# wkentaro/chainer-mask-rcnn

Hardware: AMD Instinct MI355X
Metric: images/sec train step, ResNet50-C4 Mask R-CNN, COCO 800x1333 (higher is better)
Workload: dtype f32 (bf16x3 split operands, f32 accumulate)

## Files before the change

### chainer_mask_rcnn_amd/csrc/conv_gemm.hip

```cpp
#include <algorithm>
#include <cstring>

#include "conv_gemm_kernel.h"

namespace {

__global__ void splitk_reduce_kernel(const float *__restrict__ ws, int splits, int64_t n,
                                     int64_t stride, float *__restrict__ out)
{
    const int64_t nv = n / 4;
    for (int64_t i = (int64_t)blockIdx.x * blockDim.x + threadIdx.x; i < nv;
         i += (int64_t)gridDim.x * blockDim.x) {
        float4 a = reinterpret_cast<const float4 *>(ws)[i];
        int s = 1;
        for (; s + 4 <= splits; s += 4) {
            const float4 v0 = reinterpret_cast<const float4 *>(ws + (s + 0) * stride)[i];
            const float4 v1 = reinterpret_cast<const float4 *>(ws + (s + 1) * stride)[i];
            const float4 v2 = reinterpret_cast<const float4 *>(ws + (s + 2) * stride)[i];
            const float4 v3 = reinterpret_cast<const float4 *>(ws + (s + 3) * stride)[i];
            a.x += v0.x; a.y += v0.y; a.z += v0.z; a.w += v0.w;
            a.x += v1.x; a.y += v1.y; a.z += v1.z; a.w += v1.w;
            a.x += v2.x; a.y += v2.y; a.z += v2.z; a.w += v2.w;
            a.x += v3.x; a.y += v3.y; a.z += v3.z; a.w += v3.w;
        }
// ... 214 lines not shown
                      (int64_t)d->N * d->P * d->Q * d->K < (int64_t)INT32_MAX,
                  "conv: tensor exceeds 2^31 elements");
    return 0;
}

inline bool aligned16(const void *p) { return ((uintptr_t)p % 16) == 0; }

int set_extents(GemmParams &p, int64_t a_floats, int64_t b_floats, int64_t c_floats)
{
    const int64_t lim = (int64_t)1 << 29;
    MRCNN_REQUIRE(a_floats < lim && b_floats < lim && c_floats < lim,
                  "conv: a tensor exceeds 2 GiB (%lld / %lld / %lld floats); split the batch",
                  (long long)a_floats, (long long)b_floats, (long long)c_floats);
    p.a_bytes = (unsigned)(a_floats * 4);
    p.b_bytes = (unsigned)(b_floats * 4);
    p.c_bytes = (unsigned)(c_floats * 4);
    return 0;
}


int fwd_problem(const mrcnn_conv_desc *d, GemmParams &p)
{
    if (int rc = check_desc(d)) return rc;
    p.M = d->N * d->P * d->Q; p.N = d->K; p.Kc = d->C;
    p.gp = d->P; p.gq = d->Q; p.sh = d->H; p.sw = d->W;
    p.R = d->R; p.S = d->S; p.stride = d->stride; p.pad = d->pad;
    p.lda = d->C; p.ldb = d->R * d->S * d->C; p.ldc = d->K;
    p.out_mode = OUT_PLAIN;
    p.perm_n = choose_perm(g_knobs, d->N, d->P, d->Q, d->R, d->S, d->stride, d->pad);
    if (p.perm_n) p.M = (int)(mrcnn::ceil_div(d->N, kPermBlock) * kPermBlock) * d->P * d->Q;
    return set_extents(p, (int64_t)d->N * d->H * d->W * d->C, (int64_t)d->K * d->R * d->S * d->C,
                       (int64_t)d->N * d->P * d->Q * d->K);
}

int stem_problem(int N, int H, int W, int K, GemmParams &p)
{
    MRCNN_REQUIRE(N > 0 && H > 0 && W > 0 && K > 0 && K % 4 == 0, "conv_stem: bad shape");
    const int P = (H + 6 - 7) / 2 + 1, Q = (W + 6 - 7) / 2 + 1;
    p.M = N * P * Q; p.N = K; p.Kc = 32;
    p.gp = P; p.gq = Q; p.sh = H; p.sw = W;
    p.R = 7; p.S = 1; p.stride = 2; p.pad = 3;
    p.lda = 4; p.ldb = 7 * 32; p.ldc = K;
    p.out_mode = OUT_PLAIN; p.stem = 1;
    return set_extents(p, (int64_t)N * H * W * 4, (int64_t)K * 7 * 32, (int64_t)N * P * Q * K);
}

int dgrad_problem(const mrcnn_conv_desc *d, bool fused_grad, GemmParams &p)
{
    if (int rc = check_desc(d)) return rc;
    MRCNN_REQUIRE(!fused_grad || d->stride == 1,
                  "conv2d_dgrad: residual gradient / output mask need stride 1");
    p.N = d->C; p.Kc = d->K; p.cin = d->C;
    p.R = d->R; p.S = d->S; p.pad = d->pad;
    p.lda = d->K; p.ldb = d->R * d->S * d->C; p.ldc = d->C;
    p.sh = d->P; p.sw = d->Q;
    if (d->stride == 1) {
        p.M = d->N * d->H * d->W; p.gp = d->H; p.gq = d->W; p.stride = 1;
        p.out_mode = OUT_PLAIN;
    } else {
        MRCNN_REQUIRE(d->R == 1 && d->S == 1 && d->pad == 0,
                      "conv2d_dgrad: stride>1 is implemented for 1x1/pad0 (the only strided "
                      "trainable convs of ResNet-C4) and the 2x2/2 adjoint (deconv entry points)");
        p.M = d->N * d->P * d->Q; p.gp = d->P; p.gq = d->Q; p.stride = d->stride;
        p.out_mode = OUT_STRIDED; p.oh = d->H; p.ow = d->W;
    }
    return set_extents(p, (int64_t)d->N * d->P * d->Q * d->K, (int64_t)d->K * d->R * d->S * d->C,
                       (int64_t)d->N * d->H * d->W * d->C);
}

int dgrad_wt_problem(const mrcnn_conv_desc *d, bool fused_grad, GemmParams &p)
{
    if (int rc = check_desc(d)) return rc;
    const bool strided = d->stride > 1;
    MRCNN_REQUIRE(!strided || (d->R == 1 && d->S == 1 && d->pad == 0),
                  "conv2d_dgrad_wt: stride > 1 is implemented for 1x1 / pad 0 filters");
    MRCNN_REQUIRE(!strided || !fused_grad, "conv2d_dgrad_wt: residual gradient / output mask need stride 1");
    p.N = d->C; p.Kc = d->K;
    p.sh = d->P; p.sw = d->Q;
    p.R = d->R; p.S = d->S; p.stride = 1; p.pad = d->R - 1 - d->pad;
    p.lda = d->K; p.ldb = d->R * d->S * d->K; p.ldc = d->C;
    if (strided) {
        p.gp = d->P; p.gq = d->Q; p.ostride = d->stride;
        p.out_mode = OUT_STRIDED; p.oh = d->H; p.ow = d->W;
    } else {
        p.gp = d->H; p.gq = d->W;
        p.out_mode = OUT_PLAIN;
        p.perm_n = choose_perm(g_knobs, d->N, d->H, d->W, d->R, d->S, 1, p.pad);
    }
    p.M = d->N * p.gp * p.gq;
    if (p.perm_n) p.M = (int)(mrcnn::ceil_div(d->N, kPermBlock) * kPermBlock) * d->H * d->W;
    MRCNN_REQUIRE(d->S - 1 - d->pad == p.pad, "conv2d_dgrad_wt: square filters / symmetric padding only");
    return set_extents(p, (int64_t)d->N * d->P * d->Q * d->K, (int64_t)d->K * d->R * d->S * d->C,
                       (int64_t)d->N * d->H * d->W * d->C);
}

int wgrad_problem(const mrcnn_conv_desc *d, GemmParams &p, GemmShape &shape)
{
    const int64_t pixels = (int64_t)d->N * d->P * d->Q;
    p.M = d->K; p.N = d->R * d->S * d->C; p.Kc = (int)pixels;
    p.gp = d->P; p.gq = d->Q; p.sh = d->H; p.sw = d->W;
    p.R = d->R; p.S = d->S; p.stride = d->stride; p.pad = d->pad;
    p.lda = d->C; p.ldg = d->K; p.cin = d->C; p.ldc = d->R * d->S * d->C;
    shape = gemm_shape(p, WGRAD, false);
    shape.pixels = pixels; shape.n_img = d->N; shape.C = d->C;
    return set_extents(p, pixels * d->K, (int64_t)d->N * d->H * d->W * d->C, (int64_t)d->K * d->R * d->S * d->C);
}

inline mrcnn_conv_desc deconv_adjoint_desc(int N, int H, int W, int C, int K)
{
    return {N, 2 * H, 2 * W, K, C, 2, 2, 2, 0, H, W};
}

int deconv_problem(bool wt, int N, int H, int W, int C, int K, GemmParams &p)
{
    MRCNN_REQUIRE(N > 0 && H > 0 && W > 0 && C > 0 && K > 0 && C % 4 == 0 && K % 4 == 0,
                  "%s: bad shape", wt ? "deconv_fwd_wt" : "deconv_fwd");
    p.M = N * H * W; p.N = 4 * K; p.Kc = C; p.cin = wt ? 0 : 4 * K;
    p.gp = H; p.gq = W; p.sh = H; p.sw = W;
    p.R = 1; p.S = 1; p.stride = 1; p.pad = 0;
    p.lda = C; p.ldb = wt ? C : 4 * K; p.ldc = K;
    p.out_mode = OUT_DECONV; p.ko = K;
    return set_extents(p, (int64_t)N * H * W * C, (int64_t)C * 4 * K, (int64_t)N * 4 * H * W * K);
}

int deconv_fwd(bool wt, const float *x, const float *w, const float *bias, float *y, int N, int H, int W,
               int C, int K, int epi_flags, void *stream)
{
    const char *who = wt ? "deconv_fwd_wt" : "deconv_fwd";
    GemmParams p = {};
    if (int rc = deconv_problem(wt, N, H, W, C, K, p)) return rc;
    MRCNN_REQUIRE(x && w && y, "%s: null pointer", who);
    MRCNN_REQUIRE(aligned16(x) && aligned16(w), "%s: x/%s must be 16-byte aligned", who, wt ? "wT" : "w");
    MRCNN_REQUIRE((epi_flags & ~(MRCNN_EPI_BIAS | MRCNN_EPI_RELU)) == 0, "%s: bad flags", who);
    MRCNN_REQUIRE(!(epi_flags & MRCNN_EPI_BIAS) || bias, "%s: bias flag without bias", who);
    p.A = x; p.B = w; p.C = y; p.bias = bias;
    p.flags = epi_flags;
    return wt ? launch<FWD>(p, mrcnn::as_stream(stream)) : launch<DGRAD>(p, mrcnn::as_stream(stream));
}

int wgrad_run(const mrcnn_conv_desc *d, const float *gy, const float *x, float *gw, void *ws,
              const float *out_row_scale, void *stream)
{
    GemmParams p = {};
    GemmShape shape;
    if (int rc = wgrad_problem(d, p, shape)) return rc;
    p.A = gy; p.B = x; p.C = gw;
    p.scale = out_row_scale;
    p.split_ws = (float *)ws;
    shape.has_ws = ws != nullptr;
    return run_plan<WGRAD>(p, plan_wgrad(shape, g_knobs), mrcnn::as_stream(stream));
}

extern float g_wino_ambiguity;

}

extern "C" int64_t mrcnn_conv2d_split_workspace_bytes(void) { return kSplitWsBytes; }

extern "C" int mrcnn_set_tuning(const char *name, int value)
{
    MRCNN_REQUIRE(name != nullptr, "set_tuning: null name");
    MRCNN_REQUIRE(knob_value_ok(name, value), "set_tuning: split_planes must be 1, 2 or 3, got %d (it stays %d)",
                  value, g_knobs.split_planes);
    if (set_knob(g_knobs, name, value)) return 0;
    if (strcmp(name, "wino_ambiguity_ppb") == 0) {
        g_wino_ambiguity = 1e-9f * (float)value;
        return 0;
    }
    if (int rc = mrcnn::roi_align_set_tuning(name, value); rc >= 0) return rc;
    MRCNN_REQUIRE(false, "set_tuning: unknown option '%s'", name);
    return 1;
}

extern "C" int mrcnn_conv2d_fwd(const mrcnn_conv_desc *d, const float *x, const float *w,
                                const float *bias, const float *scale, const float *shift,
                                const float *residual, float *y, int epi_flags, void *split_ws,
                                void *stream)
{
    GemmParams p = {};
    if (int rc = fwd_problem(d, p)) return rc;
    MRCNN_REQUIRE(x && w && y, "conv2d_fwd: null pointer");
    MRCNN_REQUIRE(aligned16(x) && aligned16(w), "conv2d_fwd: x/w must be 16-byte aligned");
    MRCNN_REQUIRE(!(epi_flags & MRCNN_EPI_BIAS) || bias, "conv2d_fwd: bias flag without bias");
    MRCNN_REQUIRE(!(epi_flags & MRCNN_EPI_AFFINE) || (scale && shift), "conv2d_fwd: affine flag without scale/shift");
    MRCNN_REQUIRE(!(epi_flags & MRCNN_EPI_RESIDUAL) || residual, "conv2d_fwd: residual flag without residual");
    p.A = x; p.B = w; p.C = y;
    p.bias = bias; p.scale = scale; p.shift = shift; p.residual = residual;
    p.flags = epi_flags;
    p.split_ws = (float *)split_ws;
    return launch<FWD>(p, mrcnn::as_stream(stream));
}

extern "C" int mrcnn_conv_stem_fwd(const float *x4, const float *w784, const float *bias,
                                   const float *scale, const float *shift, float *y, int N, int H,
                                   int W, int K, int epi_flags, void *stream)
{
    GemmParams p = {};
    if (int rc = stem_problem(N, H, W, K, p)) return rc;
    MRCNN_REQUIRE(x4 && w784 && y, "conv_stem: null pointer");
    MRCNN_REQUIRE(aligned16(x4) && aligned16(w784), "conv_stem: pointers must be 16-byte aligned");
    p.A = x4; p.B = w784; p.C = y;
    p.bias = bias; p.scale = scale; p.shift = shift;
    p.flags = epi_flags;
    return launch<FWD>(p, mrcnn::as_stream(stream));
}

extern "C" int mrcnn_conv2d_dgrad_ex(const mrcnn_conv_desc *d, const float *gy, const float *w,
                                     float *gx, int epi_flags, const float *res_g,
                                     const float *res_y, const float *out_mask_y,
                                     const float *out_scale, void *split_ws, void *stream)
{
    GemmParams p = {};
    if (int rc = dgrad_problem(d, res_g || out_mask_y, p)) return rc;
    MRCNN_REQUIRE(!res_y || res_g, "conv2d_dgrad: res_y without res_g");
    MRCNN_REQUIRE(gy && w && gx, "conv2d_dgrad: null pointer");
    MRCNN_REQUIRE(aligned16(gy) && aligned16(w), "conv2d_dgrad: gy/w must be 16-byte aligned");
    MRCNN_REQUIRE((epi_flags & ~MRCNN_EPI_ACCUM) == 0, "conv2d_dgrad: only MRCNN_EPI_ACCUM is valid");
    hipStream_t s = mrcnn::as_stream(stream);
    p.A = gy; p.B = w; p.C = gx;
    p.res_g = res_g; p.res_y = res_y; p.out_mask_y = out_mask_y; p.scale = out_scale;
    p.flags = epi_flags | (out_scale ? MRCNN_EPI_AFFINE : 0);
    p.split_ws = (float *)split_ws;
    if (p.out_mode == OUT_STRIDED && !(epi_flags & MRCNN_EPI_ACCUM))
        MRCNN_HIP_TRY(hipMemsetAsync(gx, 0, sizeof(float) * (size_t)d->N * d->H * d->W * d->C, s));
    return launch<DGRAD>(p, s);
}

extern "C" int mrcnn_conv2d_dgrad(const mrcnn_conv_desc *d, const float *gy, const float *w,
                                  float *gx, int epi_flags, void *stream)
{
    return mrcnn_conv2d_dgrad_ex(d, gy, w, gx, epi_flags, nullptr, nullptr, nullptr, nullptr, nullptr,
                                 stream);
}


namespace {
__global__ void filter_flip_transpose_kernel(const float *__restrict__ w, float *__restrict__ wT,
                                             int K, int RS, int C,
                                             const float *__restrict__ row_scale)
{
    __shared__ float tile[32][33];
    const int rs = blockIdx.z;
    const int k0 = blockIdx.y * 32, c0 = blockIdx.x * 32;
    const int tx = threadIdx.x & 31, ty = threadIdx.x >> 5;
    for (int j = ty; j < 32; j += 8) {
        const int k = k0 + j, c = c0 + tx;
        tile[j][tx] = (k < K && c < C)
                          ? w[((int64_t)k * RS + rs) * C + c] * (row_scale ? row_scale[k] : 1.f)
                          : 0.f;
    }
    __syncthreads();
    for (int j = ty; j < 32; j += 8) {
        const int c = c0 + j, k = k0 + tx;
        if (c < C && k < K) wT[((int64_t)c * RS + (RS - 1 - rs)) * K + k] = tile[tx][j];
    }
}

constexpr int kFlipBatch = 32;
struct FlipBatch {
    const float *w[kFlipBatch];
    float *wT[kFlipBatch];
    const float *scale[kFlipBatch];
    int K[kFlipBatch], RS[kFlipBatch], C[kFlipBatch];
    int first_block[kFlipBatch + 1];
    int n;
};

__global__ void filter_flip_transpose_batched_kernel(const FlipBatch b)
{
    __shared__ float tile[32][33];
    int l = 0;
    while (l + 1 < b.n && (int)blockIdx.x >= b.first_block[l + 1]) ++l;
    const int K = b.K[l], RS = b.RS[l], C = b.C[l];
    int blk = blockIdx.x - b.first_block[l];
    const int ncb = (C + 31) / 32, nkb = (K + 31) / 32;
    const int cb = blk % ncb;
    blk /= ncb;
    const int kb = blk % nkb, rs = blk / nkb;
    const float *__restrict__ w = b.w[l];
    float *__restrict__ wT = b.wT[l];
    const float *__restrict__ row_scale = b.scale[l];
    const int k0 = kb * 32, c0 = cb * 32;
    const int tx = threadIdx.x & 31, ty = threadIdx.x >> 5;
    for (int j = ty; j < 32; j += 8) {
        const int k = k0 + j, c = c0 + tx;
        tile[j][tx] = (k < K && c < C)
                          ? w[((int64_t)k * RS + rs) * C + c] * (row_scale ? row_scale[k] : 1.f)
                          : 0.f;
    }
    __syncthreads();
    for (int j = ty; j < 32; j += 8) {
        const int c = c0 + j, k = k0 + tx;
        if (c < C && k < K) wT[((int64_t)c * RS + (RS - 1 - rs)) * K + k] = tile[tx][j];
    }
}
}

extern "C" int mrcnn_filter_flip_transpose_batched(int n, const void *const *w, void *const *wT,
                                                   const int *K, const int *R, const int *S,
                                                   const int *C, const void *const *row_scale,
                                                   void *stream)
{
    MRCNN_REQUIRE(n >= 0 && (n == 0 || (w && wT && K && R && S && C)),
                  "filter_flip_transpose_batched: bad args");
    for (int i0 = 0; i0 < n; i0 += kFlipBatch) {
        FlipBatch b = {};
        b.n = std::min(kFlipBatch, n - i0);
        int blocks = 0;
        for (int i = 0; i < b.n; ++i) {
            const int j = i0 + i;
            MRCNN_REQUIRE(w[j] && wT[j] && K[j] > 0 && R[j] > 0 && S[j] > 0 && C[j] > 0,
                          "filter_flip_transpose_batched: bad entry %d", j);
            b.w[i] = (const float *)w[j];
            b.wT[i] = (float *)wT[j];
            b.scale[i] = row_scale ? (const float *)row_scale[j] : nullptr;
            b.K[i] = K[j]; b.RS[i] = R[j] * S[j]; b.C[i] = C[j];
            b.first_block[i] = blocks;
            blocks += ((C[j] + 31) / 32) * ((K[j] + 31) / 32) * R[j] * S[j];
        }
// ... 176 lines not shown
```

### chainer_mask_rcnn_amd/csrc/conv_winograd.h

```cpp
#pragma once

namespace {

constexpr int kXi = 36;

struct F2 { float x, y; };
__device__ __forceinline__ F2 operator+(F2 a, F2 b) { return {a.x + b.x, a.y + b.y}; }
__device__ __forceinline__ F2 operator-(F2 a, F2 b) { return {a.x - b.x, a.y - b.y}; }
__device__ __forceinline__ F2 operator*(float s, F2 a) { return {s * a.x, s * a.y}; }

template <typename T>
__device__ __forceinline__ void wino_bt(const T (&d)[6], T (&t)[6])
{
    t[0] = d[0] - 1.5f * d[1] - 2.f * d[2] + 1.5f * d[3] + d[4];
    t[1] = 2.5f * d[3] + 0.5f * d[2] - d[1] + d[4];
    t[2] = d[1] - 2.5f * d[2] + 0.5f * d[3] + d[4];
    t[3] = 2.f * (d[3] - d[1]) - d[2] + d[4];
    t[4] = 0.5f * (d[1] - d[3]) - d[2] + d[4];
    t[5] = d[1] - 1.5f * d[2] - 2.f * d[3] + 1.5f * d[4] + d[5];
}
template <typename T>
__device__ __forceinline__ void wino_at(const T (&m)[6], T (&y)[4])
{
    const T s12 = m[1] + m[2], d12 = m[1] - m[2];
    y[0] = m[0] + s12 + m[3] + m[4];
    y[1] = d12 + 0.5f * m[3] - 2.f * m[4];
    y[2] = s12 + 0.25f * m[3] + 4.f * m[4];
    y[3] = d12 + 0.125f * m[3] - 8.f * m[4] + m[5];
}
template <typename T>
__device__ __forceinline__ void wino_at_abs(const T (&m)[6], T (&y)[4])
{
    const T s12 = m[1] + m[2];
    y[0] = m[0] + s12 + m[3] + m[4];
    y[1] = s12 + 0.5f * m[3] + 2.f * m[4];
    y[2] = s12 + 0.25f * m[3] + 4.f * m[4];
    y[3] = s12 + 0.125f * m[3] + 8.f * m[4] + m[5];
}
template <typename T>
__device__ __forceinline__ void wino_g4(const T (&g)[4], T (&t)[6])
{
    t[0] = g[0];
    t[1] = g[0] + g[1] + g[2] + g[3];
    t[2] = g[1] - g[0] - g[2] + g[3];
    t[3] = -16.f * g[0] - 8.f * g[1] - 4.f * g[2] - 2.f * g[3];
    t[4] = g[0] - 2.f * g[1] + 4.f * g[2] - 8.f * g[3];
    t[5] = g[3];
}

__constant__ double kFilterG[6][3] = {{1., 0., 0.},
                                      {1. / 3, 1. / 3, 1. / 3},
                                      {-1. / 3, 1. / 3, -1. / 3},
                                      {-16. / 15, -8. / 15, -4. / 15},
                                      {1. / 15, -2. / 15, 4. / 15},
                                      {0., 0., 1.}};
__constant__ double kWgradAT[3][6] = {{1., 1. / 3, 1. / 3, 1. / 15, 1. / 15, 0.},
                                      {0., 1. / 3, -1. / 3, 1. / 30, -2. / 15, 0.},
                                      {0., 1. / 3, 1. / 3, 1. / 60, 4. / 15, 1.}};

struct WinoGeom {
    int N, H, W, TH, TW;
    int64_t T;
};
inline WinoGeom wino_geom(const mrcnn_conv_desc *d)
{
    WinoGeom g;
    g.N = d->N; g.H = d->H; g.W = d->W;
    g.TH = (d->H + 3) / 4; g.TW = (d->W + 3) / 4;
    g.T = (int64_t)d->N * g.TH * g.TW;
    return g;
}

template <bool GRAD_TILE>
__global__ void __launch_bounds__(256) wino_data_transform_kernel(
    const float *__restrict__ x, float *__restrict__ v, int H, int W, int C, int TH, int TW,
    int64_t T)
{
    constexpr int D = GRAD_TILE ? 4 : 6;
    const int c2n = C >> 1;
    const int64_t idx = (int64_t)blockIdx.x * 256 + threadIdx.x;
    if (idx >= T * c2n) return;
    const int64_t tile = idx / c2n;
    const int c = (int)(idx - tile * c2n) * 2;
    const int tx = (int)(tile % TW);
    const int64_t q = tile / TW;
    const int ty = (int)(q % TH);
    const int64_t n = q / TH;
    const int y0 = 4 * ty - (GRAD_TILE ? 0 : 1), x0 = 4 * tx - (GRAD_TILE ? 0 : 1);
    const float *base = x + (n * H * W) * C + c;
    F2 d[D][D];
#pragma unroll
    for (int i = 0; i < D; ++i)
#pragma unroll
        for (int j = 0; j < D; ++j) {
            const int yy = y0 + i, xx = x0 + j;
            const bool ok = (unsigned)yy < (unsigned)H && (unsigned)xx < (unsigned)W;
            d[i][j] = ok ? *reinterpret_cast<const F2 *>(base + ((int64_t)yy * W + xx) * C)
                         : F2{0.f, 0.f};
        }
    F2 t[6][D];
#pragma unroll
    for (int j = 0; j < D; ++j) {
        F2 col[D], o[6];
#pragma unroll
        for (int i = 0; i < D; ++i) col[i] = d[i][j];
        if constexpr (GRAD_TILE) wino_g4(col, o);
        else wino_bt(col, o);
#pragma unroll
        for (int a = 0; a < 6; ++a) t[a][j] = o[a];
    }
    float *out = v + tile * C + c;
    const int64_t xi_stride = T * C;
#pragma unroll
    for (int a = 0; a < 6; ++a) {
        F2 o[6];
        if constexpr (GRAD_TILE) wino_g4(t[a], o);
        else wino_bt(t[a], o);
#pragma unroll
        for (int b = 0; b < 6; ++b)
            *reinterpret_cast<F2 *>(out + (a * 6 + b) * xi_stride) = o[b];
    }
}

struct WinoOutParams {
    const float *m;
    float *y;
    const float *scale, *shift, *mask;
    int H, W, K, TH, TW, flags;
    int64_t T;
    int *fix_count;
    int2 *fix_list;
    int fix_cap;
    float ambiguity;
};
float g_wino_ambiguity = 4e-6f;

template <bool FIXUP>
__global__ void __launch_bounds__(256) wino_output_transform_kernel(const WinoOutParams p)
{
    const int k2n = p.K >> 1;
    const int64_t idx = (int64_t)blockIdx.x * 256 + threadIdx.x;
    if (idx >= p.T * k2n) return;
    const int64_t tile = idx / k2n;
    const int k = (int)(idx - tile * k2n) * 2;
    const int tx = (int)(tile % p.TW);
    const int64_t q = tile / p.TW;
    const int ty = (int)(q % p.TH);
    const int64_t n = q / p.TH;
    const float *in = p.m + tile * p.K + k;
    const int64_t xi_stride = p.T * p.K;
    F2 m[6][6];
#pragma unroll
    for (int a = 0; a < 6; ++a)
#pragma unroll
        for (int b = 0; b < 6; ++b)
            m[a][b] = *reinterpret_cast<const F2 *>(in + (a * 6 + b) * xi_stride);
    const int y0 = 4 * ty, x0 = 4 * tx;
    const int64_t obase = (n * p.H * p.W) * p.K + k;
    F2 mk[4][4];
    if (p.mask) {
#pragma unroll
        for (int i = 0; i < 4; ++i)
#pragma unroll
            for (int j = 0; j < 4; ++j) {
                const bool ok = y0 + i < p.H && x0 + j < p.W;
                mk[i][j] = ok ? *reinterpret_cast<const F2 *>(
                                    p.mask + obase + ((int64_t)(y0 + i) * p.W + x0 + j) * p.K)
                              : F2{0.f, 0.f};
            }
    }
    F2 s[4][6];
    F2 sa[FIXUP ? 4 : 1][6];
#pragma unroll
    for (int b = 0; b < 6; ++b) {
        F2 col[6], o[4];
#pragma unroll
        for (int a = 0; a < 6; ++a) col[a] = m[a][b];
        wino_at(col, o);
#pragma unroll
        for (int i = 0; i < 4; ++i) s[i][b] = o[i];
        if constexpr (FIXUP) {
#pragma unroll
            for (int a = 0; a < 6; ++a) col[a] = F2{fabsf(col[a].x), fabsf(col[a].y)};
            wino_at_abs(col, o);
#pragma unroll
            for (int i = 0; i < 4; ++i) sa[i][b] = o[i];
        }
    }
    F2 sc = {1.f, 1.f}, sh = {0.f, 0.f};
    const bool aff = (p.flags & (MRCNN_EPI_AFFINE | MRCNN_EPI_BIAS)) != 0;
    const bool relu = (p.flags & MRCNN_EPI_RELU) != 0;
    if (aff) {
        if (p.scale) sc = *reinterpret_cast<const F2 *>(p.scale + k);
        if (p.shift) sh = *reinterpret_cast<const F2 *>(p.shift + k);
    }
#pragma unroll
    for (int i = 0; i < 4; ++i) {
        F2 o[4], ob[4];
        wino_at(s[i], o);
        if constexpr (FIXUP) wino_at_abs(sa[i], ob);
#pragma unroll
        for (int j = 0; j < 4; ++j) {
            if (y0 + i >= p.H || x0 + j >= p.W) continue;
            F2 v = o[j];
            if (aff) { v.x = v.x * sc.x + sh.x; v.y = v.y * sc.y + sh.y; }
            if constexpr (FIXUP) {
                const float bx = p.ambiguity * ob[j].x * fabsf(sc.x);
                const float by = p.ambiguity * ob[j].y * fabsf(sc.y);
                const int pix = (int)(n * p.H * p.W) + (y0 + i) * p.W + x0 + j;
                if (fabsf(v.x) < bx) {
                    const int at = atomicAdd(p.fix_count, 1);
                    if (at < p.fix_cap) p.fix_list[at] = make_int2(pix, k);
                }
                if (fabsf(v.y) < by) {
                    const int at = atomicAdd(p.fix_count, 1);
                    if (at < p.fix_cap) p.fix_list[at] = make_int2(pix, k + 1);
                }
            }
            if (relu) { v.x = fmaxf(v.x, 0.f); v.y = fmaxf(v.y, 0.f); }
            if (p.mask) {
                v.x = mk[i][j].x > 0.f ? v.x : 0.f;
                v.y = mk[i][j].y > 0.f ? v.y : 0.f;
            }
            *reinterpret_cast<F2 *>(p.y + obase + ((int64_t)(y0 + i) * p.W + x0 + j) * p.K) = v;
        }
    }
}

struct WinoFixParams {
    const float *x, *w, *scale, *shift;
    float *y;
    const int *count;
    const int2 *list;
    int cap, H, W, C, K, flags;
};
__global__ void __launch_bounds__(256) wino_fixup_kernel(const WinoFixParams p)
{
    const int lane = threadIdx.x & 63;
    const int wave = (int)((blockIdx.x * 256 + threadIdx.x) >> 6), nwaves = (int)(gridDim.x * 4);
    const int n_items = min(*p.count, p.cap);
    for (int it = wave; it < n_items; it += nwaves) {
        const int2 e = p.list[it];
        const int pix = e.x, k = e.y;
        const int n = pix / (p.H * p.W), rem = pix - n * (p.H * p.W);
        const int yy = rem / p.W, xx = rem - yy * p.W;
        float acc = 0.f;
        for (int r = 0; r < 3; ++r) {
            const int iy = yy + r - 1;
            if ((unsigned)iy >= (unsigned)p.H) continue;
            for (int s = 0; s < 3; ++s) {
                const int ix = xx + s - 1;
                if ((unsigned)ix >= (unsigned)p.W) continue;
                const float *xp = p.x + ((int64_t)(n * p.H + iy) * p.W + ix) * p.C;
                const float *wp = p.w + ((int64_t)k * 9 + r * 3 + s) * p.C;
                for (int c = lane * 4; c < p.C; c += 256) {
                    const float4 a = *reinterpret_cast<const float4 *>(xp + c);
                    const float4 b = *reinterpret_cast<const float4 *>(wp + c);
                    acc += (a.x * b.x + a.y * b.y) + (a.z * b.z + a.w * b.w);
                }
            }
        }
#pragma unroll
        for (int off = 32; off > 0; off >>= 1) acc += __shfl_down(acc, off, 64);
        if (lane == 0) {
            float v = acc;
            if (p.flags & (MRCNN_EPI_AFFINE | MRCNN_EPI_BIAS))
                v = v * (p.scale ? p.scale[k] : 1.f) + (p.shift ? p.shift[k] : 0.f);
            if (p.flags & MRCNN_EPI_RELU) v = fmaxf(v, 0.f);
            p.y[(int64_t)pix * p.K + k] = v;
        }
    }
}

template <bool TRANSPOSED>
__global__ void __launch_bounds__(256) wino_filter_transform_kernel(
    const float *__restrict__ w, float *__restrict__ u, int K, int C,
    const float *__restrict__ row_scale)
{
    __shared__ float tile[32][33];
    const int k0 = blockIdx.y * 32, c0 = blockIdx.x * 32;
    const int tx = threadIdx.x & 31, ty = threadIdx.x >> 5;
    double f[4][9];
#pragma unroll
    for (int j = 0; j < 4; ++j) {
        const int k = k0 + ty + 8 * j, c = c0 + tx;
        const bool ok = k < K && c < C;
        const double rsc = (TRANSPOSED && row_scale && ok) ? (double)row_scale[k] : 1.0;
#pragma unroll
        for (int rs = 0; rs < 9; ++rs) {
            const int src = TRANSPOSED ? 8 - rs : rs;
            f[j][rs] = ok ? (double)w[((int64_t)k * 9 + src) * C + c] * rsc : 0.0;
        }
    }
    for (int a = 0; a < 6; ++a)
        for (int b = 0; b < 6; ++b) {
            float val[4];
#pragma unroll
            for (int j = 0; j < 4; ++j) {
                double acc = 0.0;
#pragma unroll
                for (int r = 0; r < 3; ++r) {
                    const double row = kFilterG[b][0] * f[j][r * 3] + kFilterG[b][1] * f[j][r * 3 + 1] +
                                       kFilterG[b][2] * f[j][r * 3 + 2];
                    acc += kFilterG[a][r] * row;
                }
                val[j] = (float)acc;
            }
            float *dst = u + (int64_t)(a * 6 + b) * K * C;
            if constexpr (!TRANSPOSED) {
#pragma unroll
                for (int j = 0; j < 4; ++j) {
                    const int k = k0 + ty + 8 * j, c = c0 + tx;
                    if (k < K && c < C) dst[(int64_t)k * C + c] = val[j];
                }
            } else {
                __syncthreads();
#pragma unroll
                for (int j = 0; j < 4; ++j) tile[ty + 8 * j][tx] = val[j];
                __syncthreads();
#pragma unroll
                for (int j = 0; j < 4; ++j) {
                    const int c = c0 + ty + 8 * j, k = k0 + tx;
                    if (c < C && k < K) dst[(int64_t)c * K + k] = tile[tx][ty + 8 * j];
                }
            }
        }
}

__global__ void __launch_bounds__(256) wino_wgrad_finish_kernel(
    const float *__restrict__ slabs, int splits, int64_t split_stride, float *__restrict__ gw,
    const float *__restrict__ row_scale, int K, int C)
{
    const int64_t idx = (int64_t)blockIdx.x * 256 + threadIdx.x;
    if (idx >= (int64_t)K * C) return;
    const int k = (int)(idx / C), c = (int)(idx - (int64_t)k * C);
    const int64_t kc = (int64_t)K * C;
    float du[kXi];
#pragma unroll
    for (int xi = 0; xi < kXi; ++xi) du[xi] = slabs[xi * kc + idx];
    for (int s = 1; s < splits; ++s) {
        const float *sl = slabs + s * split_stride;
#pragma unroll
        for (int xi = 0; xi < kXi; ++xi) du[xi] += sl[xi * kc + idx];
    }
    const double rsc = row_scale ? (double)row_scale[k] : 1.0;
    double t[3][6];
#pragma unroll
    for (int r = 0; r < 3; ++r)
#pragma unroll
        for (int b = 0; b < 6; ++b) {
            double acc = 0.0;
#pragma unroll
            for (int a = 0; a < 6; ++a) acc += kWgradAT[r][a] * (double)du[a * 6 + b];
            t[r][b] = acc;
        }
#pragma unroll
    for (int r = 0; r < 3; ++r)
#pragma unroll
        for (int s = 0; s < 3; ++s) {
            double acc = 0.0;
#pragma unroll
            for (int b = 0; b < 6; ++b) acc += kWgradAT[s][b] * t[r][b];
            gw[((int64_t)k * 9 + r * 3 + s) * C + c] = (float)(acc * rsc);
        }
}

int wino_check(const mrcnn_conv_desc *d, const char *who)
{
    if (int rc = check_desc(d)) return rc;
    MRCNN_REQUIRE(d->R == 3 && d->S == 3 && d->stride == 1 && d->pad == 1,
                  "%s: the Winograd path serves 3x3 / stride 1 / pad 1 only", who);
    MRCNN_REQUIRE(d->C % 4 == 0 && d->K % 4 == 0, "%s: channels must be multiples of 4", who);
    const WinoGeom g = wino_geom(d);
    MRCNN_REQUIRE(g.T * std::max(d->C, d->K) < ((int64_t)1 << 29),
                  "%s: one frequency plane exceeds 2 GiB; split the batch", who);
    return 0;
}

inline int64_t wino_u_floats(const mrcnn_conv_desc *d) { return (int64_t)kXi * d->K * d->C; }
inline int64_t wino_plane_floats(const mrcnn_conv_desc *d, int ch)
{
    return (int64_t)kXi * wino_geom(d).T * ch;
}
constexpr int kWinoMaxSplits = 8;

template <bool GRAD_TILE>
void wino_launch_data_transform(const float *x, float *v, const WinoGeom &g, int C, hipStream_t s)
{
    const int64_t n = g.T * (C / 2);
    const double in_px = (double)g.N * g.H * g.W, tiles = (double)g.T;
    mrcnn::ProfScope prof(mrcnn::PROF_WINO_TRANSFORM, 0., 4.0 * C * (in_px + 36.0 * tiles), s);
    hipLaunchKernelGGL((wino_data_transform_kernel<GRAD_TILE>),
                       dim3((unsigned)mrcnn::ceil_div(n, 256)), dim3(256), 0, s, x, v, g.H, g.W, C,
                       g.TH, g.TW, g.T);
}

int wino_batched_gemm(const float *a, const float *b, float *out, int64_t T, int N, int Kc,
                      hipStream_t s)
{
    GemmParams p = {};
    p.A = a; p.B = b; p.C = out;
    p.M = (int)T; p.N = N; p.Kc = Kc;
    p.gp = p.gq = p.sh = p.sw = 1;
    p.R = p.S = 1; p.stride = 1; p.pad = 0;
    p.lda = Kc; p.ldb = Kc; p.ldc = N;
    p.out_mode = OUT_PLAIN;
    p.batch_a = T * Kc; p.batch_b = (int64_t)N * Kc; p.batch_c = T * N;
    if (int rc = set_extents(p, T * Kc, (int64_t)N * Kc, T * N)) return rc;
    const bool big = p.M > 64 && p.N > 64;
    const int64_t tiles = big ? mrcnn::ceil_div(p.M, 128) * mrcnn::ceil_div(p.N, 128)
                              : mrcnn::ceil_div(p.M, 64) * mrcnn::ceil_div(p.N, 64);
    const double flops = 2.0 * kXi * (double)T * N * Kc;
    const double bytes = 4.0 * kXi * ((double)T * N + (double)T * Kc + (double)N * Kc);
    const int rem = p.M % 128;
    const bool two_launches = big && rem > 0 && rem <= 64 && p.M >= 256;
    const bool w8 = big && w8_ok(gemm_shape(p, FWD, false), g_knobs, kXi);
    mrcnn::ProfKernelScope prof(w8 ? mrcnn::PROF_CONV_FWD_W8 : big ? mrcnn::PROF_CONV_FWD_128 : mrcnn::PROF_CONV_FWD_64,
                                flops, bytes, two_launches && !w8 ? 2 : 1);
    if (w8) {
        launch_w8_kernel(p, mrcnn::ceil_div(p.M, kW8BM) * mrcnn::ceil_div(p.N, kW8BN), kXi, s);
    } else if (two_launches) {
        const int full = p.M - rem;
        GemmParams q = p;
        q.M = full;
        launch_kernel<2, 2, FWD>(q, (int64_t)(full / 128) * mrcnn::ceil_div(p.N, 128), 1, s, kXi);
        q.M = p.M;
        q.m_lo = full;
        launch_kernel<1, 1, FWD>(q, mrcnn::ceil_div(p.N, 64), 1, s, kXi);
    } else if (big) {
        launch_kernel<2, 2, FWD>(p, tiles, 1, s, kXi);
    } else {
        launch_kernel<1, 1, FWD>(p, tiles, 1, s, kXi);
    }
    return mrcnn::check_launch("wino_batched_gemm");
}

}

extern "C" int64_t mrcnn_conv3x3_wino_v_bytes(const mrcnn_conv_desc *d)
{
    return d ? 4 * wino_plane_floats(d, d->C) : 0;
}

extern "C" int64_t mrcnn_conv3x3_wino_workspace_bytes(const mrcnn_conv_desc *d)
{
    if (!d) return 0;
    const int64_t ch = std::max(d->C, d->K);
    return 4 * ((1 + kWinoMaxSplits) * wino_u_floats(d) + 2 * wino_plane_floats(d, (int)ch));
}

extern "C" int64_t mrcnn_conv3x3_wino_u_bytes(const mrcnn_conv_desc *d)
{
    return d ? 4 * wino_u_floats(d) : 0;
}

extern "C" int mrcnn_conv3x3_wino_filter(const mrcnn_conv_desc *d, const float *w, float *u,
                                         void *stream)
{
    if (int rc = wino_check(d, "conv3x3_wino_filter")) return rc;
    MRCNN_REQUIRE(w && u, "conv3x3_wino_filter: null pointer");
    hipLaunchKernelGGL((wino_filter_transform_kernel<false>),
                       dim3((d->C + 31) / 32, (d->K + 31) / 32), dim3(256), 0,
                       mrcnn::as_stream(stream), w, u, d->K, d->C, (const float *)nullptr);
    return mrcnn::check_launch("conv3x3_wino_filter");
}

extern "C" int mrcnn_conv3x3_wino_fwd(const mrcnn_conv_desc *d, const float *x, const float *w,
                                      const float *u_pre, const float *scale, const float *shift,
                                      float *y, int epi_flags, float *v, void *ws, void *stream)
{
    if (int rc = wino_check(d, "conv3x3_wino_fwd")) return rc;
    MRCNN_REQUIRE(x && (w || u_pre) && y && ws, "conv3x3_wino_fwd: null pointer");
    MRCNN_REQUIRE((epi_flags & ~(MRCNN_EPI_AFFINE | MRCNN_EPI_BIAS | MRCNN_EPI_RELU |
                                 MRCNN_EPI_EXACT_SIGNS)) == 0,
                  "conv3x3_wino_fwd: only AFFINE or BIAS, RELU and EXACT_SIGNS");
    MRCNN_REQUIRE(!(epi_flags & MRCNN_EPI_EXACT_SIGNS) || w,
                  "conv3x3_wino_fwd: EXACT_SIGNS needs the filter itself");
    MRCNN_REQUIRE(!(epi_flags & MRCNN_EPI_AFFINE) || scale, "conv3x3_wino_fwd: affine flag without scale");
    MRCNN_REQUIRE(!(epi_flags & MRCNN_EPI_BIAS) || (shift && !scale && !(epi_flags & MRCNN_EPI_AFFINE)),
                  "conv3x3_wino_fwd: the bias flag takes the bias in `shift` and excludes AFFINE");
    hipStream_t s = mrcnn::as_stream(stream);
    const WinoGeom g = wino_geom(d);
    float *u_ws = (float *)ws;
    float *m = u_ws + wino_u_floats(d);
    float *vbuf = v ? v : m + wino_plane_floats(d, d->K);
    const float *u = u_pre;
    if (!u) {
        hipLaunchKernelGGL((wino_filter_transform_kernel<false>),
                           dim3((d->C + 31) / 32, (d->K + 31) / 32), dim3(256), 0, s, w, u_ws, d->K,
                           d->C, (const float *)nullptr);
        u = u_ws;
    }
    wino_launch_data_transform<false>(x, vbuf, g, d->C, s);
    if (int rc = wino_batched_gemm(vbuf, u, m, g.T, d->K, d->C, s)) return rc;
    WinoOutParams o = {};
    o.m = m; o.y = y; o.scale = scale; o.shift = shift;
    o.H = d->H; o.W = d->W; o.K = d->K; o.TH = g.TH; o.TW = g.TW;
    o.flags = epi_flags & ~MRCNN_EPI_EXACT_SIGNS; o.T = g.T;
    const bool fixup = (epi_flags & MRCNN_EPI_EXACT_SIGNS) != 0;
    if (fixup) {
        float *fix = (float *)ws + wino_u_floats(d) + 2 * wino_plane_floats(d, std::max(d->C, d->K));
        o.fix_count = (int *)fix;
        o.fix_list = (int2 *)(fix + 4);
        o.fix_cap = (int)std::min<int64_t>(1 << 20, (8 * wino_u_floats(d) - 4) / 2);
        o.ambiguity = g_wino_ambiguity;
        MRCNN_HIP_TRY(hipMemsetAsync(o.fix_count, 0, 16, s));
    }
    {
        mrcnn::ProfScope prof(mrcnn::PROF_WINO_TRANSFORM, 0.,
                              4.0 * d->K * (36.0 * g.T + (double)d->N * d->H * d->W), s);
        const dim3 grid((unsigned)mrcnn::ceil_div(g.T * (d->K / 2), 256));
        if (fixup) hipLaunchKernelGGL(wino_output_transform_kernel<true>, grid, dim3(256), 0, s, o);
        else hipLaunchKernelGGL(wino_output_transform_kernel<false>, grid, dim3(256), 0, s, o);
    }
    if (fixup) {
        WinoFixParams f = {};
        f.x = x; f.w = w; f.scale = scale; f.shift = shift; f.y = y;
        f.count = o.fix_count; f.list = o.fix_list; f.cap = o.fix_cap;
        f.H = d->H; f.W = d->W; f.C = d->C; f.K = d->K; f.flags = o.flags;
        hipLaunchKernelGGL(wino_fixup_kernel, dim3(1024), dim3(256), 0, s, f);
    }
    return mrcnn::check_launch("conv3x3_wino_fwd");
}

extern "C" int mrcnn_conv3x3_wino_dgrad(const mrcnn_conv_desc *d, const float *gy, const float *w,
                                        const float *w_row_scale, float *gx,
                                        const float *out_scale, const float *out_mask_y, void *ws,
                                        void *stream)
{
    if (int rc = wino_check(d, "conv3x3_wino_dgrad")) return rc;
    MRCNN_REQUIRE(gy && w && gx && ws, "conv3x3_wino_dgrad: null pointer");
    hipStream_t s = mrcnn::as_stream(stream);
    const WinoGeom g = wino_geom(d);
    const int64_t ch = std::max(d->C, d->K);
    float *u = (float *)ws;
    float *gt = u + (1 + kWinoMaxSplits) * wino_u_floats(d);
    float *m = gt + wino_plane_floats(d, (int)ch);
    hipLaunchKernelGGL((wino_filter_transform_kernel<true>),
                       dim3((d->C + 31) / 32, (d->K + 31) / 32), dim3(256), 0, s, w, u, d->K, d->C,
                       w_row_scale);
    wino_launch_data_transform<false>(gy, gt, g, d->K, s);
    if (int rc = wino_batched_gemm(gt, u, m, g.T, d->C, d->K, s)) return rc;
    WinoOutParams o = {};
    o.m = m; o.y = gx; o.scale = out_scale; o.mask = out_mask_y;
    o.H = d->H; o.W = d->W; o.K = d->C; o.TH = g.TH; o.TW = g.TW;
    o.flags = out_scale ? MRCNN_EPI_AFFINE : 0; o.T = g.T;
    {
        mrcnn::ProfScope prof(mrcnn::PROF_WINO_TRANSFORM, 0.,
                              4.0 * d->C * (36.0 * g.T + (out_mask_y ? 2.0 : 1.0) * d->N * d->H * d->W), s);
        hipLaunchKernelGGL(wino_output_transform_kernel<false>,
                           dim3((unsigned)mrcnn::ceil_div(g.T * (d->C / 2), 256)), dim3(256), 0, s, o);
    }
    return mrcnn::check_launch("conv3x3_wino_dgrad");
}

extern "C" int mrcnn_conv3x3_wino_wgrad(const mrcnn_conv_desc *d, const float *x, const float *v,
                                        const float *gy, float *gw, const float *out_row_scale,
                                        void *ws, void *stream)
{
    if (int rc = wino_check(d, "conv3x3_wino_wgrad")) return rc;
    MRCNN_REQUIRE((x != nullptr) != (v != nullptr), "conv3x3_wino_wgrad: exactly one of x / v");
    MRCNN_REQUIRE(gy && gw && ws, "conv3x3_wino_wgrad: null pointer");
    hipStream_t s = mrcnn::as_stream(stream);
    const WinoGeom g = wino_geom(d);
    float *slabs = (float *)ws + wino_u_floats(d);
    float *gt = (float *)ws + (1 + kWinoMaxSplits) * wino_u_floats(d);
    if (!v) {
        float *vx = gt + wino_plane_floats(d, std::max(d->C, d->K));
        wino_launch_data_transform<false>(x, vx, g, d->C, s);
        v = vx;
    }
    wino_launch_data_transform<true>(gy, gt, g, d->K, s);
    GemmParams p = {};
    p.A = gt; p.B = v;
    p.M = d->K; p.N = d->C; p.Kc = (int)g.T;
    p.gp = p.gq = p.sh = p.sw = 1;
    p.R = p.S = 1; p.stride = 1; p.pad = 0;
    p.lda = d->C; p.ldg = d->K; p.cin = d->C; p.ldc = d->C;
    const int64_t kc = (int64_t)d->K * d->C;
    const bool big = p.M > 64 && p.N > 64;
    const int64_t tiles = big ? mrcnn::ceil_div(p.M, 128) * mrcnn::ceil_div(p.N, 128)
                              : mrcnn::ceil_div(p.M, 64) * mrcnn::ceil_div(p.N, 64);
    const int64_t slots = big ? (single_buffered(2, WGRAD) ? 768 : kSlotsBig) : kSlotsSmall;
    int splits = std::min(kWinoMaxSplits, wgrad_splits(tiles * kXi, g.T, slots));
    p.split_len = (int)(mrcnn::ceil_div(mrcnn::ceil_div(g.T, splits), BK) * BK);
    splits = (int)mrcnn::ceil_div(g.T, p.split_len);
    p.split_stride = kXi * kc;
    p.batch_a = g.T * d->K; p.batch_b = g.T * d->C; p.batch_c = kc;
    if (int rc = set_extents(p, g.T * d->K, g.T * d->C, kc)) return rc;
    p.C = slabs;
    {
        mrcnn::ProfKernelScope prof(big ? mrcnn::PROF_CONV_WGRAD_128 : mrcnn::PROF_CONV_WGRAD_64,
                                    2.0 * kXi * (double)kc * (double)g.T,
                                    4.0 * kXi * ((double)kc * splits + (double)g.T * (d->K + d->C)));
        if (big) launch_kernel<2, 2, WGRAD>(p, tiles, splits, s, kXi);
        else launch_kernel<1, 1, WGRAD>(p, tiles, splits, s, kXi);
    }
    hipLaunchKernelGGL(wino_wgrad_finish_kernel, dim3((unsigned)mrcnn::ceil_div(kc, 256)), dim3(256),
                       0, s, (const float *)slabs, splits, p.split_stride, gw, out_row_scale, d->K,
                       d->C);
    return mrcnn::check_launch("conv3x3_wino_wgrad");
}

extern "C" int mrcnn_conv3x3_wino_fixup_count(const mrcnn_conv_desc *d, const void *ws, void *stream,
                                              int *count)
{
    MRCNN_REQUIRE(d && ws && count, "conv3x3_wino_fixup_count: null pointer");
    const float *fix = (const float *)ws + wino_u_floats(d) +
                       2 * wino_plane_floats(d, std::max(d->C, d->K));
    MRCNN_HIP_TRY(hipMemcpyAsync(count, fix, sizeof(int), hipMemcpyDeviceToHost, mrcnn::as_stream(stream)));
    MRCNN_HIP_TRY(hipStreamSynchronize(mrcnn::as_stream(stream)));
    return 0;
}
```

Baseline: 91.75.

## Merge Winograd filter and data transforms into one launch, fold fixup counter zeroing

Combines the Winograd filter transform and the input data transform into a single kernel launch that splits its grid between the two jobs, with the heavier job placed first. It also folds the memset of the fixup counter into the data-transform kernel and rewrites the filter transform with a new blocking: a direct per-thread layout for the forward case and a shared-memory staged transpose for dgrad. The intent is to cut launch overhead and small-kernel tail effects on the conv path. The cost is more complex control flow, and a merged kernel whose shared-memory footprint may reduce occupancy for the data-transform blocks.

```diff
diff --git a/chainer_mask_rcnn_amd/csrc/conv_gemm.hip b/chainer_mask_rcnn_amd/csrc/conv_gemm.hip
--- a/chainer_mask_rcnn_amd/csrc/conv_gemm.hip
+++ b/chainer_mask_rcnn_amd/csrc/conv_gemm.hip
@@ -390,6 +390,7 @@
 }
 
 extern float g_wino_ambiguity;
+extern int g_wino_merge;
 
 }
 
@@ -403,6 +404,10 @@
     if (set_knob(g_knobs, name, value)) return 0;
     if (strcmp(name, "wino_ambiguity_ppb") == 0) {
         g_wino_ambiguity = 1e-9f * (float)value;
+        return 0;
+    }
+    if (strcmp(name, "wino_merge") == 0) {
+        g_wino_merge = value != 0;
         return 0;
     }
     if (int rc = mrcnn::roi_align_set_tuning(name, value); rc >= 0) return rc;
diff --git a/chainer_mask_rcnn_amd/csrc/conv_winograd.h b/chainer_mask_rcnn_amd/csrc/conv_winograd.h
--- a/chainer_mask_rcnn_amd/csrc/conv_winograd.h
+++ b/chainer_mask_rcnn_amd/csrc/conv_winograd.h
@@ -72,13 +72,13 @@
 }
 
 template <bool GRAD_TILE>
-__global__ void __launch_bounds__(256) wino_data_transform_kernel(
-    const float *__restrict__ x, float *__restrict__ v, int H, int W, int C, int TH, int TW,
-    int64_t T)
+__device__ __forceinline__ void wino_data_transform_block(
+    int64_t block, const float *__restrict__ x, float *__restrict__ v, int H, int W, int C, int TH,
+    int TW, int64_t T)
 {
     constexpr int D = GRAD_TILE ? 4 : 6;
     const int c2n = C >> 1;
-    const int64_t idx = (int64_t)blockIdx.x * 256 + threadIdx.x;
+    const int64_t idx = block * 256 + threadIdx.x;
     if (idx >= T * c2n) return;
     const int64_t tile = idx / c2n;
     const int c = (int)(idx - tile * c2n) * 2;
@@ -120,6 +120,15 @@
         for (int b = 0; b < 6; ++b)
             *reinterpret_cast<F2 *>(out + (a * 6 + b) * xi_stride) = o[b];
     }
+}
+
+template <bool GRAD_TILE>
+__global__ void __launch_bounds__(256) wino_data_transform_kernel(
+    const float *__restrict__ x, float *__restrict__ v, int H, int W, int C, int TH, int TW,
+    int64_t T, int *__restrict__ zero16)
+{
+    if (zero16 && blockIdx.x == 0 && threadIdx.x < 4) zero16[threadIdx.x] = 0;
+    wino_data_transform_block<GRAD_TILE>(blockIdx.x, x, v, H, W, C, TH, TW, T);
 }
 
 struct WinoOutParams {
@@ -272,59 +281,119 @@
     }
 }
 
+constexpr int kWfK = 4, kWfC = 64;
+constexpr int kWfTK = 32, kWfTC = 16;
+constexpr int kWfStageLd = kWfTC + 1;
+constexpr int kWfStageFloats = kWfTK * 9 * kWfStageLd;
+
+template <bool TRANSPOSED>
+inline int64_t wino_filter_blocks(int K, int C)
+{
+    return TRANSPOSED ? mrcnn::ceil_div(K, kWfTK) * mrcnn::ceil_div(C, kWfTC)
+                      : mrcnn::ceil_div(K, kWfK) * mrcnn::ceil_div(C, kWfC);
+}
+
+__device__ __forceinline__ void wino_filter_pair(const double (&f)[9], float *__restrict__ u,
+                                                 int64_t o, int64_t plane)
+{
+#pragma unroll
+    for (int b = 0; b < 6; ++b) {
+        double row[3];
+#pragma unroll
+        for (int r = 0; r < 3; ++r)
+            row[r] = fma(kFilterG[b][2], f[r * 3 + 2],
+                         fma(kFilterG[b][0], f[r * 3], kFilterG[b][1] * f[r * 3 + 1]));
+#pragma unroll
+        for (int a = 0; a < 6; ++a) {
+            double acc = 0.0;
+#pragma unroll
+            for (int r = 0; r < 3; ++r) acc = fma(kFilterG[a][r], row[r], acc);
+            u[(a * 6 + b) * plane + o] = (float)acc;
+        }
+    }
+}
+
+template <bool TRANSPOSED>
+__device__ __forceinline__ void wino_filter_transform_block(
+    int block, const float *__restrict__ w, float *__restrict__ u, int K, int C,
+    const float *__restrict__ row_scale, float *stage)
+{
+    const int64_t plane = (int64_t)K * C;
+    if constexpr (!TRANSPOSED) {
+        const int cx = (C + kWfC - 1) / kWfC;
+        const int by = block / cx, bx = block - by * cx;
+        const int k = by * kWfK + (threadIdx.x >> 6), c = bx * kWfC + (threadIdx.x & 63);
+        if (k >= K || c >= C) return;
+        double f[9];
+#pragma unroll
+        for (int rs = 0; rs < 9; ++rs) f[rs] = (double)w[((int64_t)k * 9 + rs) * C + c];
+        wino_filter_pair(f, u, (int64_t)k * C + c, plane);
+    } else {
+        const int cx = (C + kWfTC - 1) / kWfTC;
+        const int by = block / cx, bx = block - by * cx;
+        const int k0 = by * kWfTK, c0 = bx * kWfTC;
+        {
+            const int cc = threadIdx.x & (kWfTC - 1), r0 = threadIdx.x / kWfTC;
+            const int rows = min(kWfTK, K - k0) * 9;
+            const bool c_ok = c0 + cc < C;
+#pragma unroll
+            for (int i = 0; i < kWfTK * 9 * kWfTC / 256; ++i) {
+                const int row = r0 + i * (256 / kWfTC);
+                stage[row * kWfStageLd + cc] =
+                    (c_ok && row < rows) ? w[((int64_t)k0 * 9 + row) * C + c0 + cc] : 0.f;
+            }
+        }
+        __syncthreads();
+        const int kl = threadIdx.x & (kWfTK - 1), k = k0 + kl;
+        if (k >= K) return;
+        const double rsc = row_scale ? (double)row_scale[k] : 1.0;
+#pragma unroll 1
+        for (int j = 0; j < kWfTK * kWfTC / 256; ++j) {
+            const int cl = (threadIdx.x / kWfTK) + j * (256 / kWfTK), c = c0 + cl;
+            if (c >= C) break;
+            double f[9];
+#pragma unroll
+            for (int rs = 0; rs < 9; ++rs)
+                f[rs] = (double)stage[(kl * 9 + (8 - rs)) * kWfStageLd + cl] * rsc;
+            wino_filter_pair(f, u, (int64_t)c * K + k, plane);
+        }
+    }
+}
+
 template <bool TRANSPOSED>
 __global__ void __launch_bounds__(256) wino_filter_transform_kernel(
     const float *__restrict__ w, float *__restrict__ u, int K, int C,
     const float *__restrict__ row_scale)
 {
-    __shared__ float tile[32][33];
-    const int k0 = blockIdx.y * 32, c0 = blockIdx.x * 32;
-    const int tx = threadIdx.x & 31, ty = threadIdx.x >> 5;
-    double f[4][9];
-#pragma unroll
-    for (int j = 0; j < 4; ++j) {
-        const int k = k0 + ty + 8 * j, c = c0 + tx;
-        const bool ok = k < K && c < C;
-        const double rsc = (TRANSPOSED && row_scale && ok) ? (double)row_scale[k] : 1.0;
-#pragma unroll
-        for (int rs = 0; rs < 9; ++rs) {
-            const int src = TRANSPOSED ? 8 - rs : rs;
-            f[j][rs] = ok ? (double)w[((int64_t)k * 9 + src) * C + c] * rsc : 0.0;
-        }
-    }
-    for (int a = 0; a < 6; ++a)
-        for (int b = 0; b < 6; ++b) {
-            float val[4];
-#pragma unroll
-            for (int j = 0; j < 4; ++j) {
-                double acc = 0.0;
-#pragma unroll
-                for (int r = 0; r < 3; ++r) {
-                    const double row = kFilterG[b][0] * f[j][r * 3] + kFilterG[b][1] * f[j][r * 3 + 1] +
-                                       kFilterG[b][2] * f[j][r * 3 + 2];
-                    acc += kFilterG[a][r] * row;
-                }
-                val[j] = (float)acc;
-            }
-            float *dst = u + (int64_t)(a * 6 + b) * K * C;
-            if constexpr (!TRANSPOSED) {
-#pragma unroll
-                for (int j = 0; j < 4; ++j) {
-                    const int k = k0 + ty + 8 * j, c = c0 + tx;
-                    if (k < K && c < C) dst[(int64_t)k * C + c] = val[j];
-                }
-            } else {
-                __syncthreads();
-#pragma unroll
-                for (int j = 0; j < 4; ++j) tile[ty + 8 * j][tx] = val[j];
-                __syncthreads();
-#pragma unroll
-                for (int j = 0; j < 4; ++j) {
-                    const int c = c0 + ty + 8 * j, k = k0 + tx;
-                    if (c < C && k < K) dst[(int64_t)c * K + k] = tile[tx][ty + 8 * j];
-                }
-            }
-        }
+    __shared__ float stage[TRANSPOSED ? kWfStageFloats : 1];
+    wino_filter_transform_block<TRANSPOSED>(blockIdx.x, w, u, K, C, row_scale, stage);
+}
+
+struct WinoMergedParams {
+    const float *x;
+    float *v;
+    int H, W, C, TH, TW;
+    int64_t T;
+    const float *w, *row_scale;
+    float *u;
+    int fK, fC;
+    int first_blocks;
+    int filter_first;
+    int *zero16;
+};
+template <bool TRANSPOSED>
+__global__ void __launch_bounds__(256) wino_merged_transform_kernel(const WinoMergedParams p)
+{
+    __shared__ float stage[TRANSPOSED ? kWfStageFloats : 1];
+    int block = blockIdx.x;
+    const bool second = block >= p.first_blocks;
+    if (second) block -= p.first_blocks;
+    if (second != (p.filter_first != 0)) {
+        wino_filter_transform_block<TRANSPOSED>(block, p.w, p.u, p.fK, p.fC, p.row_scale, stage);
+    } else {
+        if (p.zero16 && block == 0 && threadIdx.x < 4) p.zero16[threadIdx.x] = 0;
+        wino_data_transform_block<false>(block, p.x, p.v, p.H, p.W, p.C, p.TH, p.TW, p.T);
+    }
 }
 
 __global__ void __launch_bounds__(256) wino_wgrad_finish_kernel(
@@ -384,15 +453,56 @@
 }
 constexpr int kWinoMaxSplits = 8;
 
+inline double wino_data_bytes(const WinoGeom &g, int C)
+{
+    return 4.0 * C * ((double)g.N * g.H * g.W + 36.0 * (double)g.T);
+}
+inline double wino_filter_bytes(int K, int C) { return 4.0 * (9.0 + kXi) * K * C; }
+
 template <bool GRAD_TILE>
-void wino_launch_data_transform(const float *x, float *v, const WinoGeom &g, int C, hipStream_t s)
+void wino_launch_data_transform(const float *x, float *v, const WinoGeom &g, int C, hipStream_t s,
+                                int *zero16 = nullptr)
 {
     const int64_t n = g.T * (C / 2);
-    const double in_px = (double)g.N * g.H * g.W, tiles = (double)g.T;
-    mrcnn::ProfScope prof(mrcnn::PROF_WINO_TRANSFORM, 0., 4.0 * C * (in_px + 36.0 * tiles), s);
+    mrcnn::ProfScope prof(mrcnn::PROF_WINO_TRANSFORM, 0., wino_data_bytes(g, C), s);
     hipLaunchKernelGGL((wino_data_transform_kernel<GRAD_TILE>),
                        dim3((unsigned)mrcnn::ceil_div(n, 256)), dim3(256), 0, s, x, v, g.H, g.W, C,
-                       g.TH, g.TW, g.T);
+                       g.TH, g.TW, g.T, zero16);
+}
+
+template <bool TRANSPOSED>
+void wino_launch_filter_transform(const float *w, float *u, int K, int C, const float *row_scale,
+                                  hipStream_t s)
+{
+    hipLaunchKernelGGL((wino_filter_transform_kernel<TRANSPOSED>),
+                       dim3((unsigned)wino_filter_blocks<TRANSPOSED>(K, C)), dim3(256), 0, s, w, u, K,
+                       C, row_scale);
+}
+
+int g_wino_merge = 1;
+
+template <bool TRANSPOSED>
+void wino_launch_transforms(const float *w, float *u, int K, int C, const float *row_scale,
+                            const float *x, float *v, const WinoGeom &g, int Cd, int *zero16,
+                            hipStream_t s)
+{
+    if (!g_wino_merge) {
+        wino_launch_filter_transform<TRANSPOSED>(w, u, K, C, row_scale, s);
+        wino_launch_data_transform<false>(x, v, g, Cd, s, zero16);
+        return;
+    }
+    const int64_t data_blocks = mrcnn::ceil_div(g.T * (Cd / 2), 256);
+    const int64_t filter_blocks = wino_filter_blocks<TRANSPOSED>(K, C);
+    const double data_bytes = wino_data_bytes(g, Cd), filter_bytes = wino_filter_bytes(K, C);
+    WinoMergedParams p = {};
+    p.x = x; p.v = v; p.H = g.H; p.W = g.W; p.C = Cd; p.TH = g.TH; p.TW = g.TW; p.T = g.T;
+    p.w = w; p.row_scale = row_scale; p.u = u; p.fK = K; p.fC = C;
+    p.filter_first = filter_bytes > data_bytes;
+    p.first_blocks = (int)(p.filter_first ? filter_blocks : data_blocks);
+    p.zero16 = zero16;
+    mrcnn::ProfScope prof(mrcnn::PROF_WINO_TRANSFORM, 0., data_bytes + filter_bytes, s);
+    hipLaunchKernelGGL((wino_merged_transform_kernel<TRANSPOSED>),
+                       dim3((unsigned)(data_blocks + filter_blocks)), dim3(256), 0, s, p);
 }
 
 int wino_batched_gemm(const float *a, const float *b, float *out, int64_t T, int N, int Kc,
@@ -459,9 +569,7 @@
 {
     if (int rc = wino_check(d, "conv3x3_wino_filter")) return rc;
     MRCNN_REQUIRE(w && u, "conv3x3_wino_filter: null pointer");
-    hipLaunchKernelGGL((wino_filter_transform_kernel<false>),
-                       dim3((d->C + 31) / 32, (d->K + 31) / 32), dim3(256), 0,
-                       mrcnn::as_stream(stream), w, u, d->K, d->C, (const float *)nullptr);
+    wino_launch_filter_transform<false>(w, u, d->K, d->C, nullptr, mrcnn::as_stream(stream));
     return mrcnn::check_launch("conv3x3_wino_filter");
 }
 
@@ -484,15 +592,6 @@
     float *u_ws = (float *)ws;
     float *m = u_ws + wino_u_floats(d);
     float *vbuf = v ? v : m + wino_plane_floats(d, d->K);
-    const float *u = u_pre;
-    if (!u) {
-        hipLaunchKernelGGL((wino_filter_transform_kernel<false>),
-                           dim3((d->C + 31) / 32, (d->K + 31) / 32), dim3(256), 0, s, w, u_ws, d->K,
-                           d->C, (const float *)nullptr);
-        u = u_ws;
-    }
-    wino_launch_data_transform<false>(x, vbuf, g, d->C, s);
-    if (int rc = wino_batched_gemm(vbuf, u, m, g.T, d->K, d->C, s)) return rc;
     WinoOutParams o = {};
     o.m = m; o.y = y; o.scale = scale; o.shift = shift;
     o.H = d->H; o.W = d->W; o.K = d->K; o.TH = g.TH; o.TW = g.TW;
@@ -504,8 +603,15 @@
         o.fix_list = (int2 *)(fix + 4);
         o.fix_cap = (int)std::min<int64_t>(1 << 20, (8 * wino_u_floats(d) - 4) / 2);
         o.ambiguity = g_wino_ambiguity;
-        MRCNN_HIP_TRY(hipMemsetAsync(o.fix_count, 0, 16, s));
-    }
+    }
+    const float *u = u_pre;
+    if (!u) {
+        wino_launch_transforms<false>(w, u_ws, d->K, d->C, nullptr, x, vbuf, g, d->C, o.fix_count, s);
+        u = u_ws;
+    } else {
+        wino_launch_data_transform<false>(x, vbuf, g, d->C, s, o.fix_count);
+    }
+    if (int rc = wino_batched_gemm(vbuf, u, m, g.T, d->K, d->C, s)) return rc;
     {
         mrcnn::ProfScope prof(mrcnn::PROF_WINO_TRANSFORM, 0.,
                               4.0 * d->K * (36.0 * g.T + (double)d->N * d->H * d->W), s);
@@ -536,10 +642,7 @@
     float *u = (float *)ws;
     float *gt = u + (1 + kWinoMaxSplits) * wino_u_floats(d);
     float *m = gt + wino_plane_floats(d, (int)ch);
-    hipLaunchKernelGGL((wino_filter_transform_kernel<true>),
-                       dim3((d->C + 31) / 32, (d->K + 31) / 32), dim3(256), 0, s, w, u, d->K, d->C,
-                       w_row_scale);
-    wino_launch_data_transform<false>(gy, gt, g, d->K, s);
+    wino_launch_transforms<true>(w, u, d->K, d->C, w_row_scale, gy, gt, g, d->K, nullptr, s);
     if (int rc = wino_batched_gemm(gt, u, m, g.T, d->C, d->K, s)) return rc;
     WinoOutParams o = {};
     o.m = m; o.y = gx; o.scale = out_scale; o.mask = out_mask_y;
```

Result: no change. 91.92 (median of 2 runs) (+0.2%).
